# mbhall88/drprg

Measured on AMD Instinct MI355X. Metric: reads/sec (+ achieved HBM GB/s) predicting on mtb index, 1/2/4/8 GPUs, higher is better.
Workload: dtype u32

## Files before the change

### drprg_amd/csrc/candidates.hip

```cpp
#include "filter_common.h"
#include "verify_lane.h"
#include <algorithm>
#include <cstdint>

namespace drprg {
namespace dev {

constexpr int VS_THREADS = 512;
constexpr int VS_PER = MAX_SLICES / VS_THREADS;
template <int KC, bool PACKED>
__global__ __launch_bounds__(VS_THREADS, 8) void verify_scan_kernel(SketchArgs a, FilterWork fw, ReadClusterArgs rc)
{
    __shared__ uint32_t s_red[3][VS_THREADS / 64];
    __shared__ uint32_t s_w[VS_THREADS / 64 + 1];
    __shared__ uint32_t s_share[2];
    __shared__ __attribute__((aligned(16))) uint32_t s_pre[MAX_SLICES + 4];
    const int tid = threadIdx.x;
    static_assert(VS_PER % 4 == 0 && MAX_SLICES % (VS_THREADS * 4) == 0, "the counts are read 16 bytes at a time");
    auto my_count = [&](int i4) -> uint4 {
        return reinterpret_cast<const uint4*>(fw.super_count + (size_t)tid * VS_PER)[i4];
    };
    uint32_t run = 0;
    uint4 v[VS_PER / 4];
#pragma unroll
// ... 318 lines not shown
                cr[u] = a.tile_rec[at];
            }
#pragma unroll
            for (int u = 0; u < 4; ++u) {
                const uint32_t i = i0 + 64u * (uint32_t)u + (uint32_t)lane;
                if (i < n) {
                    fw.cand_info[dst + i] = ci[u];
                    fw.cand_pos1[dst + i] = fw.cand_pos1[dst + i] == mark ? 0u : cp[u];
                    fw.cand_rec[dst + i] = cr[u];
                }
            }
        }
    }
}

hipError_t launch_candidate_stage(const SketchArgs& a, FilterWork& fw, const ReadClusterArgs& rc, int n_cus, hipStream_t stream, bool with_totals)
{
    fw.verify_grid = std::min<uint32_t>((uint32_t)n_cus * (uint32_t)(2048 / VS_THREADS), MAX_EX_WG);
    const dim3 grid(fw.verify_grid);
    if (a.packed) {
        if (a.k == 15) hipLaunchKernelGGL((verify_scan_kernel<15, true>), grid, dim3(VS_THREADS), 0, stream, a, fw, rc);
        else hipLaunchKernelGGL((verify_scan_kernel<0, true>), grid, dim3(VS_THREADS), 0, stream, a, fw, rc);
    } else if (a.k == 15) hipLaunchKernelGGL((verify_scan_kernel<15, false>), grid, dim3(VS_THREADS), 0, stream, a, fw, rc);
    else hipLaunchKernelGGL((verify_scan_kernel<0, false>), grid, dim3(VS_THREADS), 0, stream, a, fw, rc);
    if (with_totals) hipLaunchKernelGGL(hit_scan_kernel, dim3(1), dim3(SCAN_THREADS), 0, stream, a, fw, 0, fw.verify_grid);
    return hipGetLastError();
}

bool direct_uses_wave_form(int k, int w, bool wide_hash, bool force_lds) { return !wide_hash && !force_lds && wave_kernel_applies(k, w); }

uint32_t direct_candidate_tiles(uint64_t n_bases, int halo, int k, int w, bool wide_hash, bool force_lds)
{
    return direct_uses_wave_form(k, w, wide_hash, force_lds) ? wave_n_slices(n_bases) : sketch_n_tiles(n_bases, halo);
}

uint32_t direct_first_read_tiles(uint64_t n_bases, int halo, int k, int w, bool wide_hash, bool force_lds)
{
    return direct_uses_wave_form(k, w, wide_hash, force_lds) ? wave_n_tiles(n_bases) : sketch_n_tiles(n_bases, halo);
}

// ... 57 lines not shown
```

### drprg_amd/csrc/filter_common.h

```cpp
#pragma once
#include "common.h"
#include "device_common.h"

namespace drprg {
namespace dev {

constexpr int FT_THREADS = 1024;
constexpr int FT_WAVES = FT_THREADS / 64;
constexpr int FT_G = 32;
constexpr int FT_WPOS = 63 * FT_G;
DRPRG_HD constexpr int filter_positions_per_lane(bool level0, bool packed) { return level0 && packed ? 64 : 32; }
constexpr int FT_BLOOM_WORDS = 1 << 14;
constexpr int FT_L0_WORDS = 1 << 15;
constexpr int EX_THREADS = 256;
constexpr int SCAN_THREADS = 1024;
constexpr int MAX_SLICES = SCAN_THREADS * 8;
constexpr int FT_DEPTH = 3;
constexpr int FT_SUPER = 8;
constexpr int MAX_CHUNKS = MAX_SLICES * FT_SUPER;
constexpr int MAX_EX_WG = SCAN_THREADS * 4;

__device__ inline void candidate_range(const FilterWork& fw, uint32_t wg, uint32_t n_wg, uint32_t& t_begin, uint32_t& t_end)
{
    const uint32_t total = *fw.cand_total;
    const uint32_t per_wg = (total + n_wg - 1) / n_wg;
    const uint64_t b = (uint64_t)wg * per_wg;
    t_begin = b < total ? (uint32_t)b : total;
    t_end = b + per_wg < total ? (uint32_t)(b + per_wg) : total;
}

hipError_t launch_candidate_stage(const SketchArgs& a, FilterWork& fw, const ReadClusterArgs& rc, int n_cus, hipStream_t stream, bool with_totals = true);
hipError_t launch_read_cluster(const SketchArgs& a, const FilterWork& fw, const ReadClusterArgs& rc, int n_cus, bool skip, hipStream_t stream);

}
}
```

### drprg_amd/csrc/kernels.h

```cpp
#pragma once
#include <cstddef>
#include <cstdint>
#include <hip/hip_runtime_api.h>
#include "switches.h"

#if defined(__HIPCC__)
#define DRPRG_HD __host__ __device__
#else
#define DRPRG_HD
#endif

namespace drprg {
namespace dev {

constexpr int HIT_POS_BITS = 23;
constexpr int HIT_PRG_BITS = 12;
constexpr int HIT_READ_BITS = 28;
constexpr uint64_t HIT_POS_MASK = (1ull << HIT_POS_BITS) - 1;
constexpr uint32_t MAX_BATCH_READS = 1u << HIT_READ_BITS;
constexpr uint32_t MAX_PRGS = 1u << HIT_PRG_BITS;

DRPRG_HD inline uint64_t pack_hit_key(uint32_t read, uint32_t prg, uint32_t rev, uint32_t pos)
{
    return ((uint64_t)read << (HIT_PRG_BITS + 1 + HIT_POS_BITS)) | ((uint64_t)prg << (1 + HIT_POS_BITS))
// ... 156 lines not shown
struct ReadClusterArgs {
    const uint32_t* prg_min_path_len;
    double fraction;
    uint32_t min_cluster_size;
    int max_diff;
    uint32_t n_prgs;
    uint32_t* covg;
    uint32_t* prg_reads;
    unsigned long long* n_clusters_kept;
    unsigned long long* n_hits_kept;
    unsigned long long* n_complex;
    uint32_t* chunk_counter;
    const uint32_t* slice_prefix;
    uint32_t n_slices, mark_epoch;
    const uint32_t* block_first;
    const uint32_t *wg_hits, *wg_nmin, *wg_maxlen;
    uint32_t n_wg;
    unsigned long long *tot_hits, *tot_minimizers, *tot_max_len;
    const uint32_t* overflow_word;
    uint32_t minpath_in_lds;
};
hipError_t launch_counters_home(unsigned long long* from, unsigned long long* to, uint32_t n, hipStream_t stream, uint32_t* zero = nullptr, uint32_t n_zero = 0);
uint32_t* filter_super_counts(uint32_t* small);
uint32_t filter_super_words();
size_t filter_small_words();
void init_candidate_work(FilterWork& fw, const FilterBuffers& b, int n_cus);
hipError_t launch_sketch_filter(const SketchArgs& a, const BloomTables& bt, int n_cus, const FilterBuffers& b, const ReadClusterArgs& rc, FilterWork& fw,
    const Switches& sw, hipStream_t stream, KernelTimer timer = {});
hipError_t launch_filter_recount(const SketchArgs& a, const FilterWork& fw, hipStream_t stream);
hipError_t launch_filter_expand(const SketchArgs& a, const FilterWork& fw, hipStream_t stream);
hipError_t launch_direct_candidates(const SketchArgs& a, bool wide_hash, bool force_lds, uint32_t* tile_prefix, void* temp, size_t temp_bytes,
    uint64_t dense_capacity, const ReadClusterArgs& rc, int n_cus, FilterWork& fw, hipStream_t stream, KernelTimer timer, uint32_t slices_mark);
hipError_t launch_tile_gather_marked(const SketchArgs& a, const FilterWork& fw, const uint32_t* tile_prefix, uint32_t n_tiles, uint64_t dense_capacity,
    uint32_t mark, hipStream_t stream);
// ... 34 lines not shown
```

### drprg_amd/csrc/read_cluster.hip

```cpp
#include "filter_common.h"
#include <algorithm>
#include <cstdint>

namespace drprg {
namespace dev {

constexpr int RC_THREADS = 1024;
constexpr int RC_WAVES = RC_THREADS / 64;
constexpr int RC_PER = 2;
constexpr int RC_WG_PER_CU = 2;
constexpr int RC_SLOTS = RC_THREADS * RC_PER;
constexpr int RC_HCAP = 3072;
constexpr int RC_POOL = 512;
constexpr uint32_t RC_IRREGULAR = 2u, RC_COMPLEX = 1u;

__device__ __forceinline__ uint32_t pack_max(uint32_t earlier, uint32_t later)
{
    const uint32_t lead = (later >> 16) > (earlier >> 16) ? (later >> 16) : (earlier >> 16);
    const uint32_t seg = (later & 0xFFFFu) > (earlier & 0xFFFFu) ? (later & 0xFFFFu) : (earlier & 0xFFFFu);
    return (lead << 16) | seg;
}
__device__ __forceinline__ void lds_barrier() { asm volatile("s_waitcnt lgkmcnt(0)\n\ts_barrier" ::: "memory"); }
__device__ __forceinline__ void lds_barrier(int& t) { asm volatile("s_waitcnt lgkmcnt(0)\n\ts_barrier" : "+v"(t) : : "memory"); }

template <bool SLICES, int AHEAD>
__global__ __launch_bounds__(RC_THREADS, 4 * RC_WG_PER_CU) void read_cluster_kernel(SketchArgs a, FilterWork fw, ReadClusterArgs rc)
{
    constexpr int RC_AHEAD = AHEAD, RC_OWN = RC_SLOTS - AHEAD;
    static_assert(RC_OWN % 64 == 0, "the slices form locates 64 entries from a multiple of 64 per wave");
    (void)RC_AHEAD;
    extern __shared__ uint32_t s_hist[];
    __shared__ uint32_t s_read[RC_SLOTS + 1], s_hstart[RC_SLOTS + 1];
    __shared__ uint16_t s_pos1[RC_SLOTS];
    __shared__ uint32_t s_gt[RC_SLOTS];
    __shared__ uint16_t s_lead[RC_SLOTS];
    __shared__ uint16_t s_seg[RC_SLOTS];
    __shared__ uint16_t s_end[RC_SLOTS];
    __shared__ uint16_t s_g0[RC_SLOTS];
    __shared__ uint8_t s_dec[RC_SLOTS];
    __shared__ uint8_t s_cplx[RC_SLOTS], s_irrf[RC_SLOTS];
    __shared__ uint16_t s_grp[RC_HCAP];
    __shared__ uint16_t s_hpos[RC_HCAP];
    __shared__ uint32_t s_cov[RC_HCAP];
    __shared__ uint32_t s_w[2][RC_WAVES];
    __shared__ uint32_t s_irr[RC_POOL];
    __shared__ uint32_t s_prev_read, s_n_irr, s_chunk;
    __shared__ unsigned long long s_tot[3];

    int tid = threadIdx.x;
#define lane (tid & 63)
#define wave (tid >> 6)
    if (rc.n_wg && blockIdx.x == 0) {
        uint32_t h = 0, nm = 0, ml = 0;
        for (uint32_t g = (uint32_t)tid; g < rc.n_wg; g += RC_THREADS) {
            h += rc.wg_hits[g];
            nm += rc.wg_nmin[g];
            const uint32_t m = rc.wg_maxlen[g];
            ml = m > ml ? m : ml;
        }
        const uint32_t wh = wave_inclusive_scan(h), wn = wave_inclusive_scan(nm), wm = wave_max(ml);
        if (lane == 63) {
            s_w[0][wave] = wh;
            s_w[1][wave] = wn;
            s_irr[wave] = wm;
        }
        __syncthreads();
        if (tid == 0) {
            unsigned long long th = 0, tn = 0;
            uint32_t tm = 0;
            for (int i = 0; i < RC_WAVES; ++i) {
                th += s_w[0][i];
                tn += s_w[1][i];
                tm = s_irr[i] > tm ? s_irr[i] : tm;
            }
            *rc.tot_hits = th;
            if (tn && !(*reinterpret_cast<volatile const uint32_t*>(rc.overflow_word) & 4u)) atomicAdd(rc.tot_minimizers, tn);
            *rc.tot_max_len = (unsigned long long)tm;
        }
        __syncthreads();
    }
    if (*reinterpret_cast<volatile uint32_t*>(a.overflow) & 4u) return;
    const uint32_t total = SLICES ? rc.slice_prefix[rc.n_slices] : *fw.cand_total;
    const uint32_t handled_mark = SLICES ? rc.mark_epoch : 0u;
    uint16_t* const s_minpath = reinterpret_cast<uint16_t*>(s_hist + rc.n_prgs);
    for (uint32_t i = tid; i < rc.n_prgs; i += RC_THREADS) {
        s_hist[i] = 0;
        if (rc.minpath_in_lds) {
            const uint32_t m = rc.prg_min_path_len[i];
            s_minpath[i] = (uint16_t)(m < 0xFFFFu ? m : 0xFFFFu);
        }
    }
    if (tid < 3) s_tot[tid] = 0;
    unsigned long long my_kept_hits = 0;
    uint32_t my_kept = 0, my_complex = 0;
    const uint32_t w1_magic = w1_reciprocal(a.w);

    struct Staged {
        uint4 rec[RC_PER];
        uint32_t info[RC_PER], pos1[RC_PER], edge_prev, edge_next;
    };
    auto request = [&](uint32_t chunk) {
        Staged st;
        const uint64_t b64 = (uint64_t)chunk * RC_OWN;
        const bool live = b64 < total;
        const uint32_t b = live ? (uint32_t)b64 : 0u;
        const uint32_t n_in = total - b < (uint32_t)RC_SLOTS ? total - b : (uint32_t)RC_SLOTS;
        if constexpr (!SLICES) {
#pragma unroll
            for (int q = 0; q < RC_PER; ++q) {
                const uint32_t i = (uint32_t)tid + (uint32_t)q * RC_THREADS;
                const uint32_t src = b + (i < n_in ? i : 0u);
                st.info[q] = live ? (uint32_t)fw.cand_info[src] : 0u;
                st.pos1[q] = live ? fw.cand_pos1[src] : 0u;
                st.rec[q] = live ? fw.cand_rec[src] : make_uint4(0, 0, 0, 0);
            }
            const bool nxt = n_in == (uint32_t)RC_SLOTS && b + n_in < total;
            st.edge_prev = live ? (uint32_t)fw.cand_info[b ? b - 1 : 0u] : 0u;
            st.edge_next = live ? (uint32_t)fw.cand_info[nxt ? b + n_in : b] : 0u;
        } else {
            const uint32_t* __restrict__ P = rc.slice_prefix;
            uint32_t* const s_mine = s_gt + (wave << 6);
            const uint32_t d_last = b + n_in - 1;
            const bool nxt = n_in == (uint32_t)RC_SLOTS && b + n_in < total;
            uint32_t d0[RC_PER + 1], s0[RC_PER + 1], pj[RC_PER + 1], p0[RC_PER + 1], sn = 0, pn0 = 0;
            bool some[RC_PER + 1];
#pragma unroll
            for (int q = 0; q <= RC_PER; ++q) {
                d0[q] = q < RC_PER ? b + ((uint32_t)(wave << 6) + (uint32_t)q * RC_THREADS) : b - 64u;
                some[q] = q < RC_PER ? live && d0[q] <= d_last : live && b && wave == 0;
                s0[q] = some[q] ? rc.block_first[__builtin_amdgcn_readfirstlane(d0[q] >> 6)] : 0u;
            }
            const bool edge_n = live && nxt && wave == 0;
            if (edge_n) sn = rc.block_first[__builtin_amdgcn_readfirstlane((b + n_in) >> 6)];
// ... 54 lines not shown
    };
    auto take_ticket = [&]() -> uint32_t { return atomicAdd(rc.chunk_counter, 1u) + gridDim.x; };
    uint32_t cur = blockIdx.x;
    Staged nx = request(cur);
    for (;;) {
        lds_barrier(tid);
        const uint64_t base64 = (uint64_t)cur * RC_OWN;
        if (base64 >= total) break;
        const uint32_t base = (uint32_t)base64;
        const uint32_t n_loaded = total - base < (uint32_t)RC_SLOTS ? total - base : (uint32_t)RC_SLOTS;
        const uint32_t n_own = total - base < (uint32_t)RC_OWN ? total - base : (uint32_t)RC_OWN;
        uint32_t ticket = 0;
        if (tid == 0) ticket = take_ticket();
        uint4 crec[RC_PER];
        uint32_t st_read[RC_PER], st_pos1[RC_PER];
#pragma unroll
        for (int q = 0; q < RC_PER; ++q) {
            st_read[q] = nx.info[q];
            st_pos1[q] = nx.pos1[q];
            crec[q] = nx.rec[q];
        }
        const bool has_next = n_loaded == (uint32_t)RC_SLOTS && base + n_loaded < total;
        const uint32_t edge_prev = nx.edge_prev, edge_next = nx.edge_next;
#pragma unroll
        for (int q = 0; q < RC_PER; ++q) {
            const uint32_t i = (uint32_t)tid + (uint32_t)q * RC_THREADS;
            const bool in = i < n_loaded;
            st_read[q] = in ? st_read[q] & 0x7FFFFFFFu : READ_NONE;
            st_pos1[q] = in ? st_pos1[q] : 0u;
            if (!in) crec[q] = make_uint4(0, 0, 0, 0);
        }
#pragma unroll
        for (int q = 0; q < RC_PER; ++q) {
            const uint32_t i = (uint32_t)tid + (uint32_t)q * RC_THREADS;
            const uint32_t read = st_read[q], pos1 = st_pos1[q];
            if (!pos1) crec[q].y = 0;
            s_read[i] = read;
            s_pos1[i] = (uint16_t)(pos1 < 0xFFFFu ? pos1 : 0xFFFFu);
            s_hstart[i] = crec[q].y;
            s_g0[i] = (uint16_t)((crec[q].z >> 16) & 0x7FFFu);
            s_cplx[i] = 0;
            s_irrf[i] = 0;
        }
        if (tid == 0) {
            s_prev_read = base ? (edge_prev & 0x7FFFFFFFu) : 0xFFFFFFFFu;
            s_read[RC_SLOTS] = has_next ? (edge_next & 0x7FFFFFFFu) : 0xFFFFFFFFu;
            s_n_irr = 0;
        }
        lds_barrier(tid);
        {
            uint32_t v[RC_PER], m[RC_PER], run = 0, mx = 0;
#pragma unroll
            for (int q = 0; q < RC_PER; ++q) {
                const uint32_t i = (uint32_t)tid * RC_PER + q;
                v[q] = run;
                run += s_hstart[i];
                const uint32_t r = s_read[i], p1 = s_pos1[i];
                const uint32_t r_prev = i ? s_read[i - 1] : s_prev_read;
                if (r != r_prev) {
                    if (r != READ_NONE) mx = ((i + 1) << 16) | (i + 1);
                } else if (p1 && i) {
                    uint32_t pp = s_pos1[i - 1];
                    if (!pp) {
                        int j = (int)i - 2;
                        while (j >= 0 && s_read[j] == r && !s_pos1[j]) --j;
                        pp = (j >= 0 && s_read[j] == r) ? s_pos1[j] : p1;
                    }
                    if ((int)(p1 - pp) > rc.max_diff) mx = (mx & 0xFFFF0000u) | (i + 1);
                }
                m[q] = mx;
            }
            uint32_t incl = run, imx = mx;
#pragma unroll
            for (int off = 1; off < 64; off <<= 1) {
                const uint32_t n = __shfl_up(incl, off), x = __shfl_up(imx, off);
                if (lane >= off) {
                    incl += n;
                    imx = pack_max(x, imx);
                }
            }
            if (lane == 63) {
                s_w[0][wave] = incl;
                s_w[1][wave] = imx;
            }
            const uint32_t excl_mx_in_wave = __shfl_up(imx, 1);
            lds_barrier(tid);
            uint32_t before = incl - run, mx_before = lane ? excl_mx_in_wave : 0u, sum = 0;
#pragma unroll
            for (int i = 0; i < RC_WAVES; ++i) {
                const uint32_t x = s_w[0][i], y = s_w[1][i];
                if (i < wave) {
                    before += x;
                    mx_before = pack_max(mx_before, y);
                }
                sum += x;
            }
#pragma unroll
            for (int q = 0; q < RC_PER; ++q) {
                const uint32_t i = (uint32_t)tid * RC_PER + q;
                const uint32_t pm = pack_max(mx_before, m[q]);
// ... 57 lines not shown
        }
        lds_barrier(tid);
#pragma unroll
        for (int q = 0; q < RC_PER; ++q) {
            const uint32_t i = (uint32_t)tid + (uint32_t)q * RC_THREADS;
            const uint32_t lead = s_lead[i];
            if (i >= n_loaded || s_seg[i] != i + 1 || lead == 0 || lead > n_own) continue;
            uint32_t flags = (s_cplx[lead - 1] ? RC_COMPLEX : 0u) | (s_irrf[lead - 1] ? RC_IRREGULAR : 0u);
            bool dropped = false;
            uint32_t e = i;
            if (flags == RC_IRREGULAR) {
                for (uint32_t sg = i; sg < (uint32_t)RC_SLOTS && s_lead[sg] == lead; sg = s_end[sg]) e = s_end[sg];
                dropped = s_hstart[e] - s_hstart[lead - 1] <= rc.min_cluster_size;
            }
            if (lead == i + 1) {
                if (flags & RC_COMPLEX) ++my_complex;
                else if ((flags & RC_IRREGULAR) && !dropped) {
                    const uint32_t at = atomicAdd(&s_n_irr, 1u);
                    if (at < (uint32_t)RC_POOL) s_irr[at] = i | (e << 16);
                    else ++my_complex;
                }
            }
            const uint32_t n_hits = s_hstart[s_end[i]] - s_hstart[i];
            uint32_t dec = dropped ? 1u : 0u;
            if (!flags && n_hits) {
                const uint32_t g_thr = s_gt[i];
                dec = 1;
                if (n_hits > (g_thr & 0xFFFFu)) {
                    dec = 2;
                    atomicAdd(&s_hist[g_thr >> 17], 1u);
                    ++my_kept;
                    my_kept_hits += n_hits;
                }
            }
            s_dec[i] = (uint8_t)dec;
        }
        lds_barrier(tid);
        {
#pragma unroll
            for (int q = 0; q < RC_PER; ++q) {
                const uint32_t i = (uint32_t)tid + (uint32_t)q * RC_THREADS;
                const uint32_t lead = s_lead[i], cnt = crec[q].y;
                if (!cnt || lead == 0 || lead > n_own) continue;
                const uint32_t decision = s_dec[(uint32_t)s_seg[i] - 1];
                if (!decision) continue;
                fw.cand_pos1[base + i] = handled_mark;
                if (decision == 2) {
                    atomicAdd(&rc.covg[crec[q].w], 1u);
                    const uint32_t h0 = s_hstart[i];
                    for (uint32_t r = 1; r < cnt; ++r) atomicAdd(&rc.covg[s_cov[h0 + r]], 1u);
                }
            }
        }
        cur = s_chunk;
        nx = request(cur);
        const uint32_t n_irr = s_n_irr < (uint32_t)RC_POOL ? s_n_irr : (uint32_t)RC_POOL;
        for (uint32_t r = wave; r < n_irr; r += RC_WAVES) {
            const uint32_t i = s_irr[r] & 0xFFFFu, e = s_irr[r] >> 16;
            const uint32_t read = s_read[i], hb = s_hstart[i], he = s_hstart[e];
            const uint64_t len = a.offsets[read + 1] - a.offsets[read];
            uint32_t cl_g = 0, cl_n = 0, cl_first = 0, cl_last = 0;
            int nc = 0;
            bool complex = false;
            for (uint32_t b = hb; b < he && !complex; b += 64) {
                const uint32_t h = b + lane;
                const uint32_t hg = h < he ? s_grp[h] : 0u, hp = h < he ? s_hpos[h] : 0u;
                const bool valid = h < he;
                const uint64_t lt = (1ull << lane) - 1ull;
                uint64_t todo = __ballot(valid);
// ... 37 lines not shown
                        const uint64_t span = m & upto & ~((1ull << first_lane) - 1ull);
                        last_lane = 63 - __clzll((long long)span);
                        span_n = (uint32_t)__popcll(span);
                    }
                    const uint32_t fpos = __shfl(hp, first_lane), lpos = __shfl(hp, last_lane);
                    if (mine) {
                        cl_g = G;
                        cl_n = span_n;
                        cl_first = fpos;
                        cl_last = lpos;
                    }
                    nc += n_new;
                }
            }
            if (complex) {
                if (lane == 0) ++my_complex;
                continue;
            }
            const uint64_t expected = expected_minimizers(len, a.w, w1_magic);
            bool kept = false;
            if (lane < nc) {
                uint64_t m = rc.minpath_in_lds ? s_minpath[cl_g >> 1] : 0xFFFFu;
                if (m == 0xFFFFu) m = rc.prg_min_path_len[cl_g >> 1];
                if (expected < m) m = expected;
                const uint32_t length_based = (uint32_t)((double)m * rc.fraction);
                const uint32_t thr = length_based > rc.min_cluster_size ? length_based : rc.min_cluster_size;
                kept = cl_n > thr;
            }
            uint64_t alive = __ballot(kept);
            if (alive & (alive - 1)) {
                uint32_t rank = 0;
// ... 16 lines not shown
                            if (pn >= cn) {
                                alive &= ~(1ull << cur);
                                continue;
                            }
                            alive &= ~(1ull << prev);
                        }
                    }
                    prev = cur;
                    pg = cg;
                    pn = cn;
                    p_last = c_last;
                }
            }
            if ((alive >> lane) & 1ull) {
                atomicAdd(&s_hist[cl_g >> 1], 1u);
                ++my_kept;
                my_kept_hits += cl_n;
            }
            for (uint32_t b = hb; b < he; b += 64) {
                const uint32_t h = b + lane;
                const uint32_t hg = h < he ? s_grp[h] : 0xFFFFFFFFu, hp = h < he ? s_hpos[h] : 0u;
                for (uint64_t mm = alive; mm; mm &= mm - 1) {
                    const int o = __ffsll((long long)mm) - 1;
                    const uint32_t og = (uint32_t)__builtin_amdgcn_readlane((int)cl_g, o), of = (uint32_t)__builtin_amdgcn_readlane((int)cl_first, o),
                                   ol = (uint32_t)__builtin_amdgcn_readlane((int)cl_last, o);
                    if (hg == og && hp >= of && hp <= ol) atomicAdd(&rc.covg[s_cov[h]], 1u);
                }
            }
            for (uint32_t c = i + lane; c < e; c += 64)
                if (s_pos1[c]) fw.cand_pos1[base + c] = handled_mark;
        }
    }
    if (my_kept) atomicAdd(&s_tot[0], (unsigned long long)my_kept);
    if (my_kept_hits) atomicAdd(&s_tot[1], my_kept_hits);
    if (my_complex) atomicAdd(&s_tot[2], (unsigned long long)my_complex);
    __syncthreads();
    for (uint32_t i = tid; i < rc.n_prgs; i += RC_THREADS)
        if (s_hist[i]) atomicAdd(&rc.prg_reads[i], s_hist[i]);
    if (tid == 0) {
        if (s_tot[0]) atomicAdd(rc.n_clusters_kept, s_tot[0]);
        if (s_tot[1]) atomicAdd(rc.n_hits_kept, s_tot[1]);
        if (s_tot[2]) atomicAdd(rc.n_complex, s_tot[2]);
    }
}
#undef lane
#undef wave

constexpr int CH_THREADS = 256;
__global__ __launch_bounds__(CH_THREADS) void counters_home_kernel(unsigned long long* from, unsigned long long* to, uint32_t n, uint4* zero, uint32_t n_zero4)
{
    const uint32_t i = threadIdx.x;
    if (i < n) {
        to[i] = from[i];
        from[i] = 0;
    }
    for (uint32_t j = i; j < n_zero4; j += CH_THREADS) zero[j] = make_uint4(0, 0, 0, 0);
}
// ... 9 lines not shown
    if (*n_hits) *n_complex = 1;
}

hipError_t launch_read_cluster(const SketchArgs& a, const FilterWork& fw, const ReadClusterArgs& rc, int n_cus, bool skip, hipStream_t stream)
{
    if (skip) {
        hipLaunchKernelGGL(flag_complex_kernel, dim3(1), dim3(1), 0, stream, a.n_hits, rc.n_complex);
        return hipGetLastError();
    }
    ReadClusterArgs rcd = rc;
    size_t dyn = (size_t)rc.n_prgs * sizeof(uint32_t);
    {
        static size_t static_lds = 0;
        if (!static_lds) {
            size_t most = 0;
            for (const void* k : { reinterpret_cast<const void*>(&read_cluster_kernel<false, 128>), reinterpret_cast<const void*>(&read_cluster_kernel<false, 256>),
                     reinterpret_cast<const void*>(&read_cluster_kernel<false, 512>), reinterpret_cast<const void*>(&read_cluster_kernel<true, 128>),
                     reinterpret_cast<const void*>(&read_cluster_kernel<true, 256>), reinterpret_cast<const void*>(&read_cluster_kernel<true, 512>) }) {
                hipFuncAttributes at {};
                HIP_TRY(hipFuncGetAttributes(&at, k));
                most = std::max<size_t>(most, at.sharedSizeBytes);
            }
            static_lds = most;
        }
        const size_t lds_cu = 160 * 1024, with = dyn + (size_t)rc.n_prgs * sizeof(uint16_t);
        const size_t fit_without = std::min<size_t>(lds_cu / (static_lds + dyn), RC_WG_PER_CU), fit_with = std::min<size_t>(lds_cu / (static_lds + with), RC_WG_PER_CU);
        rcd.minpath_in_lds = fit_with == fit_without ? 1u : 0u;
        if (rcd.minpath_in_lds) dyn = with;
    }
    const uint64_t mean_len = a.n_bases / (a.n_reads ? a.n_reads : 1u);
    const int ahead = mean_len <= 300 ? 128 : mean_len <= 600 ? 256 : 512;
    static size_t configured[6][MAX_HIP_DEVICES] = {};
    auto launch = [&](auto kernel, size_t (&conf)[MAX_HIP_DEVICES]) -> hipError_t {
        HIP_TRY(ensure_dynamic_lds(reinterpret_cast<const void*>(kernel), dyn, conf));
        hipLaunchKernelGGL(kernel, dim3((uint32_t)n_cus * RC_WG_PER_CU), dim3(RC_THREADS), dyn, stream, a, fw, rcd);
        return hipGetLastError();
    };
    if (rcd.slice_prefix) {
        if (ahead == 128) HIP_TRY(launch(&read_cluster_kernel<true, 128>, configured[0]));
        else if (ahead == 256) HIP_TRY(launch(&read_cluster_kernel<true, 256>, configured[1]));
        else HIP_TRY(launch(&read_cluster_kernel<true, 512>, configured[2]));
    } else {
        if (ahead == 128) HIP_TRY(launch(&read_cluster_kernel<false, 128>, configured[3]));
        else if (ahead == 256) HIP_TRY(launch(&read_cluster_kernel<false, 256>, configured[4]));
        else HIP_TRY(launch(&read_cluster_kernel<false, 512>, configured[5]));
    }
    return hipGetLastError();
}

}
}
```

### drprg_amd/csrc/sketch_filter.hip

```cpp
#include "filter_common.h"
#include <algorithm>
#include <cstdint>
#include <type_traits>

namespace drprg {
namespace dev {

__device__ inline uint32_t pack16le(const uint4& in)
{
    constexpr uint32_t W = 0x40100401u;
    const uint32_t p0 = __builtin_amdgcn_udot4(in.x & 0x06060606u, W, 0u, false), p1 = __builtin_amdgcn_udot4(in.y & 0x06060606u, W, 0u, false);
    const uint32_t p2 = __builtin_amdgcn_udot4(in.z & 0x06060606u, W, 0u, false), p3 = __builtin_amdgcn_udot4(in.w & 0x06060606u, W, 0u, false);
    return ((p0 | (p1 << 8) | (p2 << 16)) >> 1) | (p3 << 23);
}


typedef __attribute__((address_space(3))) const uint32_t lds_cu32;
__device__ __forceinline__ uint32_t lds_at(uint32_t byte_addr) { return *(lds_cu32*)(uintptr_t)byte_addr; }
__device__ __forceinline__ uint32_t bloom_test(uint32_t word, uint32_t h, uint32_t x)
{
    uint32_t t2;
    asm("v_lshlrev_b32_sdwa %0, %1, %2 dst_sel:DWORD dst_unused:UNUSED_PAD src0_sel:BYTE_1 src1_sel:DWORD" : "=v"(t2) : "v"(h), "v"(word));
    return (word << (h & 31)) & t2 & (word << ((x >> 16) & 0xFF));
}
// ... 614 lines not shown
        const Kernel packed = which == 5 ? &sketch_filter_kernel<false, true, true, 2, true>
            : which == 4                 ? &sketch_filter_kernel<false, true, true, 1, true>
            : which == 3                 ? &sketch_filter_kernel<false, true, true, 3, true>
            : which == 2                 ? &sketch_filter_kernel<false, true, true, 0, true>
            : which == 1                 ? &sketch_filter_kernel<true, false, false, 0, true>
                                         : &sketch_filter_kernel<false, false, false, 0, true>;
        const Kernel kernel = a.packed ? packed : ascii;
        const size_t dyn = level0 ? (size_t)FT_L0_WORDS * 4 + (size_t)FT_WAVES * 2048 : ((size_t)4 << bt.bloom_wbits) + 16;
        fw.sched.lds_word = (uint32_t)(dyn / 4 - 4);
        static size_t configured[12][MAX_HIP_DEVICES] = {};
        HIP_TRY(ensure_dynamic_lds(reinterpret_cast<const void*>(kernel), dyn, configured[which + (a.packed ? 6 : 0)]));
        launch_timed(timer, kernel, dim3(grid), dim3(FT_THREADS), dyn, stream, a, fw);
    }
    HIP_TRY(hipGetLastError());
    const bool skip_rc = sw.skip_read_cluster;
    HIP_TRY(launch_candidate_stage(a, fw, rc, n_cus, stream, skip_rc));
    ReadClusterArgs rct = rc;
    if (!skip_rc) {
        rct.wg_hits = fw.wg_hits;
        rct.wg_nmin = fw.wg_nmin;
        rct.wg_maxlen = fw.wg_maxlen;
        rct.n_wg = fw.verify_grid;
        rct.tot_hits = a.n_hits;
        rct.tot_minimizers = a.n_minimizers;
        rct.tot_max_len = fw.max_len;
        rct.overflow_word = a.overflow;
    }
    return launch_read_cluster(a, fw, rct, n_cus, skip_rc, stream);
}

}
}
```

Before: 21.09 billion.

## Fuse candidate verification into the read-cluster kernel, dropping the separate verify-scan stage

The sketch-filter path no longer launches verify_scan and the totals scan before read clustering. The read-cluster kernel now locates each candidate's raw position itself, by scanning superblock and slice counts and binary-searching prefixes held in LDS. It verifies candidates in-lane, writes cand_info and cand_rec, and accumulates hit, minimizer and max-length totals with block atomics. This removes a kernel launch and the global write-then-reread of candidate records, at the cost of more register and LDS pressure and more complex per-chunk work in the clustering kernel. Per-thread counters are replaced by shared atomics in the fused variants.

```diff
diff --git a/drprg_amd/csrc/candidates.hip b/drprg_amd/csrc/candidates.hip
--- a/drprg_amd/csrc/candidates.hip
+++ b/drprg_amd/csrc/candidates.hip
@@ -356,7 +356,7 @@
     }
 }
 
-hipError_t launch_candidate_stage(const SketchArgs& a, FilterWork& fw, const ReadClusterArgs& rc, int n_cus, hipStream_t stream, bool with_totals)
+hipError_t launch_candidate_stage(const SketchArgs& a, FilterWork& fw, const ReadClusterArgs& rc, int n_cus, hipStream_t stream)
 {
     fw.verify_grid = std::min<uint32_t>((uint32_t)n_cus * (uint32_t)(2048 / VS_THREADS), MAX_EX_WG);
     const dim3 grid(fw.verify_grid);
@@ -365,7 +365,7 @@
         else hipLaunchKernelGGL((verify_scan_kernel<0, true>), grid, dim3(VS_THREADS), 0, stream, a, fw, rc);
     } else if (a.k == 15) hipLaunchKernelGGL((verify_scan_kernel<15, false>), grid, dim3(VS_THREADS), 0, stream, a, fw, rc);
     else hipLaunchKernelGGL((verify_scan_kernel<0, false>), grid, dim3(VS_THREADS), 0, stream, a, fw, rc);
-    if (with_totals) hipLaunchKernelGGL(hit_scan_kernel, dim3(1), dim3(SCAN_THREADS), 0, stream, a, fw, 0, fw.verify_grid);
+    hipLaunchKernelGGL(hit_scan_kernel, dim3(1), dim3(SCAN_THREADS), 0, stream, a, fw, 0, fw.verify_grid);
     return hipGetLastError();
 }
 
diff --git a/drprg_amd/csrc/filter_common.h b/drprg_amd/csrc/filter_common.h
--- a/drprg_amd/csrc/filter_common.h
+++ b/drprg_amd/csrc/filter_common.h
@@ -29,7 +29,7 @@
     t_end = b + per_wg < total ? (uint32_t)(b + per_wg) : total;
 }
 
-hipError_t launch_candidate_stage(const SketchArgs& a, FilterWork& fw, const ReadClusterArgs& rc, int n_cus, hipStream_t stream, bool with_totals = true);
+hipError_t launch_candidate_stage(const SketchArgs& a, FilterWork& fw, const ReadClusterArgs& rc, int n_cus, hipStream_t stream);
 hipError_t launch_read_cluster(const SketchArgs& a, const FilterWork& fw, const ReadClusterArgs& rc, int n_cus, bool skip, hipStream_t stream);
 
 }
diff --git a/drprg_amd/csrc/kernels.h b/drprg_amd/csrc/kernels.h
--- a/drprg_amd/csrc/kernels.h
+++ b/drprg_amd/csrc/kernels.h
@@ -194,10 +194,6 @@
     const uint32_t* slice_prefix;
     uint32_t n_slices, mark_epoch;
     const uint32_t* block_first;
-    const uint32_t *wg_hits, *wg_nmin, *wg_maxlen;
-    uint32_t n_wg;
-    unsigned long long *tot_hits, *tot_minimizers, *tot_max_len;
-    const uint32_t* overflow_word;
     uint32_t minpath_in_lds;
 };
 hipError_t launch_counters_home(unsigned long long* from, unsigned long long* to, uint32_t n, hipStream_t stream, uint32_t* zero = nullptr, uint32_t n_zero = 0);
diff --git a/drprg_amd/csrc/read_cluster.hip b/drprg_amd/csrc/read_cluster.hip
--- a/drprg_amd/csrc/read_cluster.hip
+++ b/drprg_amd/csrc/read_cluster.hip
@@ -1,6 +1,8 @@
 #include "filter_common.h"
+#include "verify_lane.h"
 #include <algorithm>
 #include <cstdint>
+#include <type_traits>
 
 namespace drprg {
 namespace dev {
@@ -23,19 +25,26 @@
 __device__ __forceinline__ void lds_barrier() { asm volatile("s_waitcnt lgkmcnt(0)\n\ts_barrier" ::: "memory"); }
 __device__ __forceinline__ void lds_barrier(int& t) { asm volatile("s_waitcnt lgkmcnt(0)\n\ts_barrier" : "+v"(t) : : "memory"); }
 
-template <bool SLICES, int AHEAD>
+template <bool SLICES, int AHEAD, int FUSE>
 __global__ __launch_bounds__(RC_THREADS, 4 * RC_WG_PER_CU) void read_cluster_kernel(SketchArgs a, FilterWork fw, ReadClusterArgs rc)
 {
     constexpr int RC_AHEAD = AHEAD, RC_OWN = RC_SLOTS - AHEAD;
     static_assert(RC_OWN % 64 == 0, "the slices form locates 64 entries from a multiple of 64 per wave");
+    static_assert(SLICES != (FUSE != 0), "the candidates come from the direct kernel's slices or from this kernel's own verification");
+    constexpr int FZ_PER = MAX_SLICES / RC_THREADS, FZ_PAIRS = MAX_SLICES / 2;
+    static_assert(FZ_PER == 8 && FT_SUPER == 8, "two 16-byte loads of counts per thread; sixteen slices per pair of superblocks");
+    constexpr int FZ_KC = (FUSE == 1 || FUSE == 3) ? 15 : 0;
+    constexpr bool FZ_PACKED = FUSE >= 3;
     (void)RC_AHEAD;
     extern __shared__ uint32_t s_hist[];
     __shared__ uint32_t s_read[RC_SLOTS + 1], s_hstart[RC_SLOTS + 1];
     __shared__ uint16_t s_pos1[RC_SLOTS];
-    __shared__ uint32_t s_gt[RC_SLOTS];
-    __shared__ uint16_t s_lead[RC_SLOTS];
-    __shared__ uint16_t s_seg[RC_SLOTS];
-    __shared__ uint16_t s_end[RC_SLOTS];
+    __shared__ __attribute__((aligned(16))) uint32_t s_zone[RC_SLOTS * 5 / 2];
+    static_assert(FZ_PAIRS + 1 <= RC_SLOTS * 5 / 2, "the pair prefixes fit the block");
+    uint32_t* const s_gt = s_zone;
+    uint16_t* const s_lead = reinterpret_cast<uint16_t*>(s_zone + RC_SLOTS);
+    uint16_t* const s_seg = s_lead + RC_SLOTS;
+    uint16_t* const s_end = s_seg + RC_SLOTS;
     __shared__ uint16_t s_g0[RC_SLOTS];
     __shared__ uint8_t s_dec[RC_SLOTS];
     __shared__ uint8_t s_cplx[RC_SLOTS], s_irrf[RC_SLOTS];
@@ -44,43 +53,32 @@
     __shared__ uint32_t s_cov[RC_HCAP];
     __shared__ uint32_t s_w[2][RC_WAVES];
     __shared__ uint32_t s_irr[RC_POOL];
-    __shared__ uint32_t s_prev_read, s_n_irr, s_chunk;
-    __shared__ unsigned long long s_tot[3];
+    __shared__ uint32_t s_prev_read, s_n_irr, s_chunk, s_share[2], s_vmax;
+    __shared__ unsigned long long s_tot[5];
 
     int tid = threadIdx.x;
 #define lane (tid & 63)
 #define wave (tid >> 6)
-    if (rc.n_wg && blockIdx.x == 0) {
-        uint32_t h = 0, nm = 0, ml = 0;
-        for (uint32_t g = (uint32_t)tid; g < rc.n_wg; g += RC_THREADS) {
-            h += rc.wg_hits[g];
-            nm += rc.wg_nmin[g];
-            const uint32_t m = rc.wg_maxlen[g];
-            ml = m > ml ? m : ml;
-        }
-        const uint32_t wh = wave_inclusive_scan(h), wn = wave_inclusive_scan(nm), wm = wave_max(ml);
-        if (lane == 63) {
-            s_w[0][wave] = wh;
-            s_w[1][wave] = wn;
-            s_irr[wave] = wm;
-        }
-        __syncthreads();
-        if (tid == 0) {
-            unsigned long long th = 0, tn = 0;
-            uint32_t tm = 0;
-            for (int i = 0; i < RC_WAVES; ++i) {
-                th += s_w[0][i];
-                tn += s_w[1][i];
-                tm = s_irr[i] > tm ? s_irr[i] : tm;
-            }
-            *rc.tot_hits = th;
-            if (tn && !(*reinterpret_cast<volatile const uint32_t*>(rc.overflow_word) & 4u)) atomicAdd(rc.tot_minimizers, tn);
-            *rc.tot_max_len = (unsigned long long)tm;
-        }
+    if (*reinterpret_cast<volatile uint32_t*>(a.overflow) & 4u) return;
+    uint32_t fz_before = 0, fz_total = 0;
+    if constexpr (FUSE != 0) {
+        const uint4* __restrict__ sc = reinterpret_cast<const uint4*>(fw.super_count + (size_t)tid * FZ_PER);
+        const uint4 c0 = sc[0], c1 = sc[1];
+        const uint32_t run = c0.x + c0.y + c0.z + c0.w + c1.x + c1.y + c1.z + c1.w;
+        fz_before = block_exclusive_scan<RC_WAVES>(run, &s_w[0][0], &fz_total);
+        fz_total = (uint32_t)__builtin_amdgcn_readfirstlane((int)fz_total);
+        if (blockIdx.x == 0 && tid == 0) *fw.cand_count = fz_total;
         __syncthreads();
     }
-    if (*reinterpret_cast<volatile uint32_t*>(a.overflow) & 4u) return;
-    const uint32_t total = SLICES ? rc.slice_prefix[rc.n_slices] : *fw.cand_total;
+    auto uni32 = [](uint32_t x) -> uint32_t { return (uint32_t)__builtin_amdgcn_readfirstlane((int)x); };
+    auto uni64 = [&](uint64_t x) -> uint64_t { return ((uint64_t)uni32((uint32_t)(x >> 32)) << 32) | (uint64_t)uni32((uint32_t)x); };
+    VerifyConsts vc(a, fw);
+    vc.w1_magic = uni32(vc.w1_magic);
+    vc.win_lo = (int64_t)uni64((uint64_t)vc.win_lo);
+    vc.win_hi = (int64_t)uni64((uint64_t)vc.win_hi);
+    vc.reads_per_base = __longlong_as_double((long long)uni64((uint64_t)__double_as_longlong(vc.reads_per_base)));
+    (void)fz_before;
+    const uint32_t total = FUSE != 0 ? fz_total : rc.slice_prefix[rc.n_slices];
     const uint32_t handled_mark = SLICES ? rc.mark_epoch : 0u;
     uint16_t* const s_minpath = reinterpret_cast<uint16_t*>(s_hist + rc.n_prgs);
     for (uint32_t i = tid; i < rc.n_prgs; i += RC_THREADS) {
@@ -90,14 +88,27 @@
             s_minpath[i] = (uint16_t)(m < 0xFFFFu ? m : 0xFFFFu);
         }
     }
-    if (tid < 3) s_tot[tid] = 0;
+    if (tid < 5) s_tot[tid] = 0;
+    if (tid == 0) s_vmax = 0;
     unsigned long long my_kept_hits = 0;
     uint32_t my_kept = 0, my_complex = 0;
-    const uint32_t w1_magic = w1_reciprocal(a.w);
+    auto count_complex = [&]() {
+        if constexpr (FUSE != 0) atomicAdd(&s_tot[2], 1ull);
+        else ++my_complex;
+    };
+    const uint32_t w1_magic = FUSE != 0 ? vc.w1_magic : w1_reciprocal(a.w);
 
     struct Staged {
-        uint4 rec[RC_PER];
+        uint4 rec[SLICES ? RC_PER : 1];
         uint32_t info[RC_PER], pos1[RC_PER], edge_prev, edge_next;
+    };
+    auto read_at = [&](int64_t gp) -> uint32_t {
+        if (!(gp >= vc.win_lo && gp < vc.win_hi && gp + vc.k <= vc.n_bases)) return READ_NONE;
+        uint32_t guess = (uint32_t)((double)gp * vc.reads_per_base);
+        if (guess >= a.n_reads) guess = a.n_reads - 1;
+        const uint64_t o0 = a.offsets[guess], o1 = a.offsets[guess + 1];
+        if (o0 <= (uint64_t)gp && (uint64_t)gp < o1) return guess;
+        return find_read_near(a.offsets, a.n_reads, guess, (uint64_t)gp);
     };
     auto request = [&](uint32_t chunk) {
         Staged st;
@@ -107,16 +118,50 @@
         const uint32_t n_in = total - b < (uint32_t)RC_SLOTS ? total - b : (uint32_t)RC_SLOTS;
         if constexpr (!SLICES) {
 #pragma unroll
-            for (int q = 0; q < RC_PER; ++q) {
-                const uint32_t i = (uint32_t)tid + (uint32_t)q * RC_THREADS;
-                const uint32_t src = b + (i < n_in ? i : 0u);
-                st.info[q] = live ? (uint32_t)fw.cand_info[src] : 0u;
-                st.pos1[q] = live ? fw.cand_pos1[src] : 0u;
-                st.rec[q] = live ? fw.cand_rec[src] : make_uint4(0, 0, 0, 0);
-            }
-            const bool nxt = n_in == (uint32_t)RC_SLOTS && b + n_in < total;
-            st.edge_prev = live ? (uint32_t)fw.cand_info[b ? b - 1 : 0u] : 0u;
-            st.edge_next = live ? (uint32_t)fw.cand_info[nxt ? b + n_in : b] : 0u;
+            for (int q = 0; q < RC_PER; ++q) st.info[q] = st.pos1[q] = 0u;
+            st.edge_prev = st.edge_next = 0u;
+            if (live) {
+                const bool nxt = n_in == (uint32_t)RC_SLOTS && b + n_in < total;
+                const uint4* __restrict__ sc = reinterpret_cast<const uint4*>(fw.super_count + (size_t)tid * FZ_PER);
+                const uint4 c0 = sc[0], c1 = sc[1];
+                const uint32_t p0 = fz_before, p1 = p0 + c0.x + c0.y, p2 = p1 + c0.z + c0.w, p3 = p2 + c1.x + c1.y, p4 = p3 + c1.z + c1.w;
+                uint32_t* const s_pre = s_zone;
+                reinterpret_cast<uint4*>(s_pre)[tid] = make_uint4(p0, p1, p2, p3);
+                if (tid == RC_THREADS - 1) s_pre[FZ_PAIRS] = p4;
+                const uint32_t x0 = b ? b - 1u : 0u, x1 = nxt ? b + n_in : b + n_in - 1u;
+                if (p0 <= x0 && x0 < p4) s_share[0] = (uint32_t)tid * 4u + (p1 <= x0 ? 1u : 0u) + (p2 <= x0 ? 1u : 0u) + (p3 <= x0 ? 1u : 0u);
+                if (p0 <= x1 && x1 < p4) s_share[1] = (uint32_t)tid * 4u + (p1 <= x1 ? 1u : 0u) + (p2 <= x1 ? 1u : 0u) + (p3 <= x1 ? 1u : 0u);
+                lds_barrier(tid);
+                const uint32_t s_lo = (uint32_t)__builtin_amdgcn_readfirstlane((int)s_share[0]), s_hi = (uint32_t)__builtin_amdgcn_readfirstlane((int)s_share[1]);
+                const uint32_t span_step = s_hi > s_lo ? 1u << (31 - __builtin_clz(s_hi - s_lo)) : 1u;
+                auto position_of = [&](uint32_t t) -> uint64_t {
+                    uint32_t lo = s_lo;
+                    for (uint32_t step = span_step; step >= 1; step >>= 1)
+                        if (lo + step <= s_hi && s_pre[lo + step] <= t) lo += step;
+                    const uint4* __restrict__ c4 = reinterpret_cast<const uint4*>(fw.slice_count) + (size_t)lo * 4;
+                    const uint4 ca = c4[0], cb = c4[1], cc = c4[2], cd = c4[3];
+                    const uint32_t cnt[15] = { ca.x, ca.y, ca.z, ca.w, cb.x, cb.y, cb.z, cb.w, cc.x, cc.y, cc.z, cc.w, cd.x, cd.y, cd.z };
+                    const uint32_t rest = t - s_pre[lo];
+                    uint32_t sum = 0, before = 0, idx = 0;
+#pragma unroll
+                    for (int u = 0; u < 15; ++u) {
+                        sum += cnt[u];
+                        const bool past = rest >= sum;
+                        idx = past ? (uint32_t)u + 1u : idx;
+                        before = past ? sum : before;
+                    }
+                    const uint32_t at = fw.slice_base[lo * 16u + idx];
+                    return fw.raw_pos[(size_t)at + (rest - before)];
+                };
+#pragma unroll
+                for (int q = 0; q < RC_PER; ++q) {
+                    const uint32_t i = (uint32_t)tid + (uint32_t)q * RC_THREADS;
+                    const uint64_t gp = position_of(b + (i < n_in ? i : 0u));
+                    st.info[q] = (uint32_t)gp;
+                    st.pos1[q] = (uint32_t)(gp >> 32);
+                }
+                if ((tid == 0 && b) || (tid == 64 && nxt)) st.edge_prev = read_at((int64_t)position_of(tid == 0 ? b - 1u : b + n_in));
+            }
         } else {
             const uint32_t* __restrict__ P = rc.slice_prefix;
             uint32_t* const s_mine = s_gt + (wave << 6);
@@ -201,27 +246,61 @@
         if (tid == 0) ticket = take_ticket();
         uint4 crec[RC_PER];
         uint32_t st_read[RC_PER], st_pos1[RC_PER];
-#pragma unroll
-        for (int q = 0; q < RC_PER; ++q) {
-            st_read[q] = nx.info[q];
-            st_pos1[q] = nx.pos1[q];
-            crec[q] = nx.rec[q];
-        }
         const bool has_next = n_loaded == (uint32_t)RC_SLOTS && base + n_loaded < total;
         const uint32_t edge_prev = nx.edge_prev, edge_next = nx.edge_next;
-#pragma unroll
-        for (int q = 0; q < RC_PER; ++q) {
-            const uint32_t i = (uint32_t)tid + (uint32_t)q * RC_THREADS;
-            const bool in = i < n_loaded;
-            st_read[q] = in ? st_read[q] & 0x7FFFFFFFu : READ_NONE;
-            st_pos1[q] = in ? st_pos1[q] : 0u;
-            if (!in) crec[q] = make_uint4(0, 0, 0, 0);
+        if constexpr (FUSE != 0) {
+            uint32_t* const s_park = s_zone + tid;
+            s_park[0] = nx.info[1];
+            s_park[RC_THREADS] = nx.pos1[1];
+            int64_t gp = (int64_t)(((uint64_t)nx.pos1[0] << 32) | (uint64_t)nx.info[0]);
+#pragma unroll
+            for (int q = 0; q < RC_PER; ++q) {
+                const uint32_t i = (uint32_t)tid + (uint32_t)q * RC_THREADS;
+                VerifyOut o;
+                uint32_t h = 0, nm = 0, ml = 0;
+                if (i < n_loaded) verify_one_lane<FZ_KC, FZ_PACKED>(a, rc, vc, gp, o, h, nm, ml);
+                if (i < n_own) {
+                    fw.cand_info[base + i] = ((uint64_t)o.slot << 32) | ((uint64_t)o.strand << 31) | (uint64_t)o.read;
+                    fw.cand_rec[base + i] = o.crec;
+                    if (nm) {
+                        atomicAdd(&s_tot[3], (unsigned long long)h);
+                        atomicAdd(&s_tot[4], 1ull);
+                        atomicMax(&s_vmax, ml);
+                    }
+                }
+                st_read[q] = o.read;
+                st_pos1[q] = o.pos1;
+                crec[q] = o.crec;
+                if (q == 0) {
+                    s_park[2 * RC_THREADS] = o.read;
+                    s_park[3 * RC_THREADS] = o.pos1;
+                    s_park[4 * RC_THREADS] = o.crec.x;
+                    s_read[i] = o.crec.y;
+                    s_hstart[i] = o.crec.z;
+                    s_cov[tid] = o.crec.w;
+                    gp = (int64_t)(((uint64_t)s_park[RC_THREADS] << 32) | (uint64_t)s_park[0]);
+                    asm volatile("" ::: "memory");
+                }
+            }
+            asm volatile("" ::: "memory");
+            st_read[0] = s_park[2 * RC_THREADS];
+            st_pos1[0] = s_park[3 * RC_THREADS];
+            crec[0] = make_uint4(s_park[4 * RC_THREADS], s_read[tid], s_hstart[tid], s_cov[tid]);
+        } else {
+#pragma unroll
+            for (int q = 0; q < RC_PER; ++q) {
+                const uint32_t i = (uint32_t)tid + (uint32_t)q * RC_THREADS;
+                const bool in = i < n_loaded;
+                st_read[q] = in ? nx.info[q] & 0x7FFFFFFFu : READ_NONE;
+                st_pos1[q] = in ? nx.pos1[q] : 0u;
+                crec[q] = in ? nx.rec[q] : make_uint4(0, 0, 0, 0);
+                if (!st_pos1[q]) crec[q].y = 0;
+            }
         }
 #pragma unroll
         for (int q = 0; q < RC_PER; ++q) {
             const uint32_t i = (uint32_t)tid + (uint32_t)q * RC_THREADS;
             const uint32_t read = st_read[q], pos1 = st_pos1[q];
-            if (!pos1) crec[q].y = 0;
             s_read[i] = read;
             s_pos1[i] = (uint16_t)(pos1 < 0xFFFFu ? pos1 : 0xFFFFu);
             s_hstart[i] = crec[q].y;
@@ -231,8 +310,12 @@
         }
         if (tid == 0) {
             s_prev_read = base ? (edge_prev & 0x7FFFFFFFu) : 0xFFFFFFFFu;
-            s_read[RC_SLOTS] = has_next ? (edge_next & 0x7FFFFFFFu) : 0xFFFFFFFFu;
+            if constexpr (FUSE == 0) s_read[RC_SLOTS] = has_next ? (edge_next & 0x7FFFFFFFu) : 0xFFFFFFFFu;
             s_n_irr = 0;
+        }
+        if constexpr (FUSE != 0) {
+            (void)edge_next;
+            if (tid == 64) s_read[RC_SLOTS] = has_next ? edge_prev : 0xFFFFFFFFu;
         }
         lds_barrier(tid);
         {
@@ -258,9 +341,13 @@
                 m[q] = mx;
             }
             uint32_t incl = run, imx = mx;
+            auto shfl_up_ = [&](uint32_t v, int off) -> uint32_t {
+                if constexpr (FUSE != 0) return (uint32_t)__builtin_amdgcn_ds_bpermute((int)(((uint32_t)lane - (uint32_t)off) << 2), (int)v);
+                else return __shfl_up(v, off);
+            };
 #pragma unroll
             for (int off = 1; off < 64; off <<= 1) {
-                const uint32_t n = __shfl_up(incl, off), x = __shfl_up(imx, off);
+                const uint32_t n = shfl_up_(incl, off), x = shfl_up_(imx, off);
                 if (lane >= off) {
                     incl += n;
                     imx = pack_max(x, imx);
@@ -270,7 +357,7 @@
                 s_w[0][wave] = incl;
                 s_w[1][wave] = imx;
             }
-            const uint32_t excl_mx_in_wave = __shfl_up(imx, 1);
+            const uint32_t excl_mx_in_wave = shfl_up_(imx, 1);
             lds_barrier(tid);
             uint32_t before = incl - run, mx_before = lane ? excl_mx_in_wave : 0u, sum = 0;
 #pragma unroll
@@ -358,11 +445,13 @@
                 dropped = s_hstart[e] - s_hstart[lead - 1] <= rc.min_cluster_size;
             }
             if (lead == i + 1) {
-                if (flags & RC_COMPLEX) ++my_complex;
+                if (flags & RC_COMPLEX) count_complex();
                 else if ((flags & RC_IRREGULAR) && !dropped) {
                     const uint32_t at = atomicAdd(&s_n_irr, 1u);
-                    if (at < (uint32_t)RC_POOL) s_irr[at] = i | (e << 16);
-                    else ++my_complex;
+                    if (at < (uint32_t)RC_POOL) {
+                        s_irr[at] = i | (e << 16);
+                        if constexpr (FUSE != 0) s_irrf[i] = 2;
+                    } else count_complex();
                 }
             }
             const uint32_t n_hits = s_hstart[s_end[i]] - s_hstart[i];
@@ -373,8 +462,13 @@
                 if (n_hits > (g_thr & 0xFFFFu)) {
                     dec = 2;
                     atomicAdd(&s_hist[g_thr >> 17], 1u);
-                    ++my_kept;
-                    my_kept_hits += n_hits;
+                    if constexpr (FUSE != 0) {
+                        atomicAdd(&s_tot[0], 1ull);
+                        atomicAdd(&s_tot[1], (unsigned long long)n_hits);
+                    } else {
+                        ++my_kept;
+                        my_kept_hits += n_hits;
+                    }
                 }
             }
             s_dec[i] = (uint8_t)dec;
@@ -385,10 +479,23 @@
             for (int q = 0; q < RC_PER; ++q) {
                 const uint32_t i = (uint32_t)tid + (uint32_t)q * RC_THREADS;
                 const uint32_t lead = s_lead[i], cnt = crec[q].y;
-                if (!cnt || lead == 0 || lead > n_own) continue;
-                const uint32_t decision = s_dec[(uint32_t)s_seg[i] - 1];
-                if (!decision) continue;
-                fw.cand_pos1[base + i] = handled_mark;
+                uint32_t decision;
+                if constexpr (FUSE != 0) {
+                    if (i >= n_loaded || lead > n_own) continue;
+                    if (lead == 0) {
+                        if (i >= (uint32_t)RC_AHEAD || base == 0) fw.cand_pos1[base + i] = st_pos1[q];
+                        continue;
+                    }
+                    if (s_irrf[lead - 1] == 2) continue;
+                    decision = cnt ? s_dec[(uint32_t)s_seg[i] - 1] : 0u;
+                    fw.cand_pos1[base + i] = decision ? 0u : st_pos1[q];
+                    if (!decision) continue;
+                } else {
+                    if (!cnt || lead == 0 || lead > n_own) continue;
+                    decision = s_dec[(uint32_t)s_seg[i] - 1];
+                    if (!decision) continue;
+                    fw.cand_pos1[base + i] = handled_mark;
+                }
                 if (decision == 2) {
                     atomicAdd(&rc.covg[crec[q].w], 1u);
                     const uint32_t h0 = s_hstart[i];
@@ -397,6 +504,8 @@
             }
         }
         cur = s_chunk;
+        if constexpr (FUSE != 0) cur = uni32(cur);
+        if constexpr (FUSE != 0) lds_barrier(tid);
         nx = request(cur);
         const uint32_t n_irr = s_n_irr < (uint32_t)RC_POOL ? s_n_irr : (uint32_t)RC_POOL;
         for (uint32_t r = wave; r < n_irr; r += RC_WAVES) {
@@ -464,7 +573,9 @@
                 }
             }
             if (complex) {
-                if (lane == 0) ++my_complex;
+                if (lane == 0) count_complex();
+                if constexpr (FUSE != 0)
+                    for (uint32_t c = i + lane; c < e; c += 64) fw.cand_pos1[base + c] = s_pos1[c];
                 continue;
             }
             const uint64_t expected = expected_minimizers(len, a.w, w1_magic);
@@ -511,8 +622,13 @@
             }
             if ((alive >> lane) & 1ull) {
                 atomicAdd(&s_hist[cl_g >> 1], 1u);
-                ++my_kept;
-                my_kept_hits += cl_n;
+                if constexpr (FUSE != 0) {
+                    atomicAdd(&s_tot[0], 1ull);
+                    atomicAdd(&s_tot[1], (unsigned long long)cl_n);
+                } else {
+                    ++my_kept;
+                    my_kept_hits += cl_n;
+                }
             }
             for (uint32_t b = hb; b < he; b += 64) {
                 const uint32_t h = b + lane;
@@ -525,7 +641,7 @@
                 }
             }
             for (uint32_t c = i + lane; c < e; c += 64)
-                if (s_pos1[c]) fw.cand_pos1[base + c] = handled_mark;
+                if (FUSE != 0 || s_pos1[c]) fw.cand_pos1[base + c] = handled_mark;
         }
     }
     if (my_kept) atomicAdd(&s_tot[0], (unsigned long long)my_kept);
@@ -538,6 +654,11 @@
         if (s_tot[0]) atomicAdd(rc.n_clusters_kept, s_tot[0]);
         if (s_tot[1]) atomicAdd(rc.n_hits_kept, s_tot[1]);
         if (s_tot[2]) atomicAdd(rc.n_complex, s_tot[2]);
+        if constexpr (FUSE != 0) {
+            if (s_tot[3]) atomicAdd(a.n_hits, s_tot[3]);
+            if (s_tot[4]) atomicAdd(a.n_minimizers, s_tot[4]);
+            if (s_vmax) atomicMax(fw.max_len, (unsigned long long)s_vmax);
+        }
     }
 }
 #undef lane
@@ -577,9 +698,9 @@
         static size_t static_lds = 0;
         if (!static_lds) {
             size_t most = 0;
-            for (const void* k : { reinterpret_cast<const void*>(&read_cluster_kernel<false, 128>), reinterpret_cast<const void*>(&read_cluster_kernel<false, 256>),
-                     reinterpret_cast<const void*>(&read_cluster_kernel<false, 512>), reinterpret_cast<const void*>(&read_cluster_kernel<true, 128>),
-                     reinterpret_cast<const void*>(&read_cluster_kernel<true, 256>), reinterpret_cast<const void*>(&read_cluster_kernel<true, 512>) }) {
+            for (const void* k : { reinterpret_cast<const void*>(&read_cluster_kernel<false, 128, 1>), reinterpret_cast<const void*>(&read_cluster_kernel<false, 256, 1>),
+                     reinterpret_cast<const void*>(&read_cluster_kernel<false, 512, 1>), reinterpret_cast<const void*>(&read_cluster_kernel<true, 128, 0>),
+                     reinterpret_cast<const void*>(&read_cluster_kernel<true, 256, 0>), reinterpret_cast<const void*>(&read_cluster_kernel<true, 512, 0>) }) {
                 hipFuncAttributes at {};
                 HIP_TRY(hipFuncGetAttributes(&at, k));
                 most = std::max<size_t>(most, at.sharedSizeBytes);
@@ -593,20 +714,29 @@
     }
     const uint64_t mean_len = a.n_bases / (a.n_reads ? a.n_reads : 1u);
     const int ahead = mean_len <= 300 ? 128 : mean_len <= 600 ? 256 : 512;
-    static size_t configured[6][MAX_HIP_DEVICES] = {};
+    static size_t configured[15][MAX_HIP_DEVICES] = {};
     auto launch = [&](auto kernel, size_t (&conf)[MAX_HIP_DEVICES]) -> hipError_t {
         HIP_TRY(ensure_dynamic_lds(reinterpret_cast<const void*>(kernel), dyn, conf));
         hipLaunchKernelGGL(kernel, dim3((uint32_t)n_cus * RC_WG_PER_CU), dim3(RC_THREADS), dyn, stream, a, fw, rcd);
         return hipGetLastError();
     };
     if (rcd.slice_prefix) {
-        if (ahead == 128) HIP_TRY(launch(&read_cluster_kernel<true, 128>, configured[0]));
-        else if (ahead == 256) HIP_TRY(launch(&read_cluster_kernel<true, 256>, configured[1]));
-        else HIP_TRY(launch(&read_cluster_kernel<true, 512>, configured[2]));
+        if (ahead == 128) HIP_TRY(launch(&read_cluster_kernel<true, 128, 0>, configured[0]));
+        else if (ahead == 256) HIP_TRY(launch(&read_cluster_kernel<true, 256, 0>, configured[1]));
+        else HIP_TRY(launch(&read_cluster_kernel<true, 512, 0>, configured[2]));
     } else {
-        if (ahead == 128) HIP_TRY(launch(&read_cluster_kernel<false, 128>, configured[3]));
-        else if (ahead == 256) HIP_TRY(launch(&read_cluster_kernel<false, 256>, configured[4]));
-        else HIP_TRY(launch(&read_cluster_kernel<false, 512>, configured[5]));
+        if (a.k > 15 || a.w > 16) return hipErrorInvalidValue;
+        const int fuse = 1 + (a.k == 15 ? 0 : 1) + (a.packed ? 2 : 0);
+        auto by_ahead = [&](auto f) -> hipError_t {
+            constexpr int F = decltype(f)::value;
+            if (ahead == 128) return launch(&read_cluster_kernel<false, 128, F>, configured[3 * F]);
+            if (ahead == 256) return launch(&read_cluster_kernel<false, 256, F>, configured[3 * F + 1]);
+            return launch(&read_cluster_kernel<false, 512, F>, configured[3 * F + 2]);
+        };
+        if (fuse == 1) HIP_TRY(by_ahead(std::integral_constant<int, 1>()));
+        else if (fuse == 2) HIP_TRY(by_ahead(std::integral_constant<int, 2>()));
+        else if (fuse == 3) HIP_TRY(by_ahead(std::integral_constant<int, 3>()));
+        else HIP_TRY(by_ahead(std::integral_constant<int, 4>()));
     }
     return hipGetLastError();
 }
diff --git a/drprg_amd/csrc/sketch_filter.hip b/drprg_amd/csrc/sketch_filter.hip
--- a/drprg_amd/csrc/sketch_filter.hip
+++ b/drprg_amd/csrc/sketch_filter.hip
@@ -652,20 +652,9 @@
     }
     HIP_TRY(hipGetLastError());
     const bool skip_rc = sw.skip_read_cluster;
-    HIP_TRY(launch_candidate_stage(a, fw, rc, n_cus, stream, skip_rc));
-    ReadClusterArgs rct = rc;
-    if (!skip_rc) {
-        rct.wg_hits = fw.wg_hits;
-        rct.wg_nmin = fw.wg_nmin;
-        rct.wg_maxlen = fw.wg_maxlen;
-        rct.n_wg = fw.verify_grid;
-        rct.tot_hits = a.n_hits;
-        rct.tot_minimizers = a.n_minimizers;
-        rct.tot_max_len = fw.max_len;
-        rct.overflow_word = a.overflow;
-    }
-    return launch_read_cluster(a, fw, rct, n_cus, skip_rc, stream);
-}
-
-}
-}
+    if (skip_rc) HIP_TRY(launch_candidate_stage(a, fw, rc, n_cus, stream));
+    return launch_read_cluster(a, fw, rc, n_cus, skip_rc, stream);
+}
+
+}
+}
```

New measurement: 20.17 billion. -4.4%, worse.
